# neptune-ai/open-solution-mapping-challenge

Measured on NVIDIA H100. Metric: 300x300 tiles/sec fwd+bwd ResNet101-UNet, higher is better.
Workload: dtype bf16

## Files before the change

### open-solution-mapping-challenge_b200/csrc/conv_gemm.cu

```cuda
#include "host_common.h"
#include "conv_gemm.cuh"
#include "../../include/mcb200.h"
#include <algorithm>
#include <mutex>
#include <stdlib.h>

namespace mcb {

static void pick_tile(int Wv, int Hv, int N, int max_rows, int row_mult, int* pbw, int* pbh, int* pbn) {
  double best = -1.0;
  int bbw = 1, bbh = 1, bbn = 1;
  for (int bw = 1; bw <= std::min(max_rows, std::min(Wv, 256)); ++bw) {
    for (int bh = 1; bw * bh <= max_rows && bh <= std::min(Hv, 256); ++bh) {
      const int bn_max = std::min(256, max_rows / (bw * bh));
      for (int bn = 1; bn <= bn_max; ++bn) {
        if (bn > N && row_mult == 1) break;
        const int rows = bw * bh * bn;
        if (rows % row_mult != 0) continue;
        const long tiles = (long)((Wv + bw - 1) / bw) * ((Hv + bh - 1) / bh) * ((N + bn - 1) / bn);
        const double eff = (double)Wv * Hv * N / ((double)tiles * max_rows);
        const double score = eff + 1e-6 * bw + 1e-9 * bh;
        if (score > best) {
          best = score;
          bbw = bw; bbh = bh; bbn = bn;
        }
      }
    }
  }
  *pbw = bbw; *pbh = bbh; *pbn = bbn;
}

constexpr int kSmemBudget = 227 * 1024;
constexpr int kMaxStagesHalo = 9, kMaxStages = 6;
constexpr int kTwoStagingMinStages = 3;
constexpr int kHaloMinChannels = 128;
constexpr int kBn256MinWaveX10 = 6;
constexpr int kWgradWavesX10 = 10;
constexpr int kWgradMinKb = 6;
constexpr int kWgradKbTarget = 64;
constexpr int kWgradMinWaveX10 = 4;

struct TestHooks { int force_bn, halo, wgrad_splits; };
static TestHooks test_hooks() {
  auto get = [](const char* name, int dflt) {
    const char* v = getenv(name);
    return v ? atoi(v) : dflt;
  };
  return {get("MCB_FORCE_BN", 0), get("MCB_HALO", 2), get("MCB_WGRAD_SPLITS", 0)};
}

template <int BN, int BK, bool B_MN, bool HALO>
static int launch_conv_inst(const ConvGemmParams& p, dim3 grid, size_t smem, cudaStream_t st) {
  static bool attr_set = false;
  if (!attr_set) {
    MCB_CHECK_CUDA(cudaFuncSetAttribute(conv_gemm_kernel<BN, BK, B_MN, HALO>,
                                        cudaFuncAttributeMaxDynamicSharedMemorySize, kSmemBudget));
    attr_set = true;
  }
  conv_gemm_kernel<BN, BK, B_MN, HALO><<<grid, kConvThreads, smem, st>>>(p);
  MCB_LAUNCH_CHECK();
  return MCB_OK;
}

template <int BK, bool B_MN, bool HALO>
static int launch_conv_bn(int BN, const ConvGemmParams& p, dim3 grid, size_t smem, cudaStream_t st) {
  switch (BN) {
    case 256: return launch_conv_inst<256, BK, B_MN, HALO>(p, grid, smem, st);
    case 128: return launch_conv_inst<128, BK, B_MN, HALO>(p, grid, smem, st);
    case 64: return launch_conv_inst<64, BK, B_MN, HALO>(p, grid, smem, st);
    case 32: return launch_conv_inst<32, BK, B_MN, HALO>(p, grid, smem, st);
  }
  return fail(MCB_ERR_UNSUPPORTED, "unsupported BN %d", BN);
}

static int launch_conv(int BN, int BK, bool b_mn, ConvGemmParams& p, int m_tiles, int n_tiles, int phases,
                       cudaStream_t st, bool halo = false) {
  const int a_bytes = halo ? ((kHaloW * kHaloH * BK * 2 + 1023) / 1024) * 1024 : 128 * BK * 2;
  const int b_bytes = BN * BK * 2;
  const int stage = halo ? b_bytes : a_bytes + b_bytes;
  const int out_buf_bytes = 128 * BN * 2;
  const int aux_bytes = p.aux_mode != 0 ? 2 * 128 * (BN >= 64 ? 64 : 32) * 2 : 0;
  const int base = aux_bytes + kStatBytes + 1024  + 1536  + (halo ? 2 * a_bytes : 0);
  const int out_bufs = (kSmemBudget - base - 2 * out_buf_bytes) / stage >= kTwoStagingMinStages ? 2 : 1;
  const int fixed = base + out_bufs * out_buf_bytes;
  const int stages = std::max(2, std::min(halo ? kMaxStagesHalo : kMaxStages, (kSmemBudget - fixed) / stage));
  p.stages = stages;
  p.out_bufs = out_bufs;
  p.m_tiles = m_tiles; p.n_tiles = n_tiles; p.phases = phases;
  const size_t smem = (size_t)stages * stage + fixed;
  const long total = (long)m_tiles * n_tiles * phases;
  dim3 grid((unsigned)std::min<long>(total, num_sms()), 1, 1);
  const int nch = n_tiles * BN;
  const bool red = p.stats != nullptr || p.aux_mode == 2 || (p.aux_mode == 1 && p.bn_dbeta != nullptr);
  p.red_stride = 2 * nch;
  if (red && (long)grid.x * p.red_stride > kConvRedCap)
    return fail(MCB_ERR_UNSUPPORTED, "conv: reduction rows %u x %d exceed the workspace", grid.x, p.red_stride);
  int r;
  if (halo) {
    if (BK == 64) r = b_mn ? launch_conv_bn<64, true, true>(BN, p, grid, smem, st) : launch_conv_bn<64, false, true>(BN, p, grid, smem, st);
    else r = b_mn ? launch_conv_bn<32, true, true>(BN, p, grid, smem, st) : launch_conv_bn<32, false, true>(BN, p, grid, smem, st);
  } else {
    if (BK == 64) r = b_mn ? launch_conv_bn<64, true, false>(BN, p, grid, smem, st) : launch_conv_bn<64, false, false>(BN, p, grid, smem, st);
    else r = b_mn ? launch_conv_bn<32, true, false>(BN, p, grid, smem, st) : launch_conv_bn<32, false, false>(BN, p, grid, smem, st);
  }
  if (r || !red) return r;
  const int rows = (int)grid.x;
  if (p.aux_mode == 0) {
    conv_red_finish_kernel<<<det_finish_grid(2L * nch, rows), kDetFinishThreads, 0, st>>>(
        0L, rows, (long)p.red_stride, 2L * nch, (long)nch, p.stats + p.n_off, (long)p.stats_c);
  } else {
    conv_red_finish_kernel<<<det_finish_grid(nch, rows), kDetFinishThreads, 0, st>>>(
        0L, rows, (long)p.red_stride, (long)nch, (long)nch, p.bn_dbeta + p.n_off, 0L);
    if (p.aux_mode == 2)
      conv_red_finish_kernel<<<det_finish_grid(nch, rows), kDetFinishThreads, 0, st>>>(
          (long)nch, rows, (long)p.red_stride, (long)nch, (long)nch, p.bn_dgamma + p.n_off, 0L);
  }
  MCB_LAUNCH_CHECK();
  return MCB_OK;
}

static bool use_halo(int ksize, int stride, int W, int H, int k_channels) {
  const int mode = test_hooks().halo;
  if (ksize != 3 || stride != 1 || mode == 0) return false;
  if (mode == 2) return k_channels >= kHaloMinChannels && W % 8 == 0 && H % 16 == 0 && W >= 80;
  const double eff = (double)W * H / ((double)((W + 7) / 8) * 8 * ((H + 15) / 16) * 16);
  return eff >= 0.8;
}

static int pick_bn(int n_total, long m_tiles, int phases) {
  int bn = 32;
  for (int cand : {256, 128, 64, 32}) {
    if (n_total % cand == 0) { bn = cand; break; }
  }
  const long sms = num_sms();
  if (bn > 128 && m_tiles * phases * (n_total / bn) * 10 < sms * kBn256MinWaveX10) bn = 128;
  if (bn > 64 && n_total % 64 == 0 && m_tiles * phases * (n_total / bn) < sms / 3) bn = 64;
  const int forced = test_hooks().force_bn;
// ... 340 lines not shown
```

### open-solution-mapping-challenge_b200/csrc/conv_gemm.cuh

```cuda
#pragma once
#include "tc.cuh"
#include "detsum.cuh"

namespace mcb {

constexpr int kMaxTaps = 24;

constexpr long kConvRedCap = 256L * 4096;
constexpr int kWgradRegions = 4;
constexpr long kWgradRegionCap = 4L * 1024 * 1024;
MCB_DET_WORKSPACE(float, g_conv_red, kConvRedCap, conv_red_finish_kernel)
MCB_DET_WORKSPACE(float, g_wgrad_red, kWgradRegions * kWgradRegionCap, wgrad_red_finish_kernel)
constexpr int kGemmThreads = 384;
constexpr int kProducerRegs = 40, kMmaRegs = 232;

struct TapDesc {
  int16_t src;
  int16_t dx, dy;
  int16_t nchunks;
  int32_t wk0;
  int32_t wtap;
};

struct ConvGemmParams {
// ... 32 lines not shown
struct WgradTap {
  int16_t srcA, ax, ay;
  int16_t srcB, bx, by;
  int32_t wtap;
};

struct WgradParams {
  CUtensorMap tmA[4];
  CUtensorMap tmB[4];
  WgradTap taps[16];
  int ntaps;
  int Wv, Hv, Nimg;
  int bw, bh, bn, rows;
  int tiles_x, tiles_y, tiles_total;
  int splits;
  int stages;
  float* dw;
  int cout, cin_total, ci_off;
  int a_cw;
  int a_chunks;
  int cin_src;
  long slice;
  long ws_off;
};

__device__ __forceinline__ uint8_t* align_up_1024(uint8_t* p) {
  const uint32_t a = static_cast<uint32_t>(__cvta_generic_to_shared(p));
  return p + ((1024u - (a & 1023u)) & 1023u);
}


constexpr int kConvThreads = 512;
constexpr int kConvProducerRegs = 24, kConvEpilogueRegs = 120, kConvMmaRegs = 184;

constexpr int kHaloW = 10, kHaloH = 18;

constexpr int kStatBytes = 4 * 8 * 16 * 4;

__device__ __forceinline__ void epi_wg_sync() { asm volatile("bar.sync 1, 128;" ::: "memory"); }

template <int BN, int BK, bool B_MN, bool HALO>
__global__ void __launch_bounds__(kConvThreads, 1) conv_gemm_kernel(const __grid_constant__ ConvGemmParams p) {
  static_assert(BK == 64 || BK == 32, "BK");
  static_assert(BN == 32 || BN == 64 || BN == 128 || BN == 256, "BN");
  constexpr int A_ROW_BYTES = BK * 2;
  constexpr int A_BYTES = HALO ? ((kHaloW * kHaloH * A_ROW_BYTES + 1023) / 1024) * 1024 : 128 * A_ROW_BYTES;
  constexpr int B_BYTES = BN * BK * 2;
  constexpr int STAGE_BYTES = HALO ? B_BYTES : A_BYTES + B_BYTES;
  constexpr int A_RING_BYTES = HALO ? 2 * A_BYTES : 0;
  constexpr uint32_t A_LAYOUT = (BK == 64) ? tc::LAYOUT_SW128 : tc::LAYOUT_SW64;
  constexpr int BMN_CW = (BN >= 64) ? 64 : 32;
  constexpr int BMN_ROW_BYTES = BMN_CW * 2;
  constexpr int BMN_SUB_BYTES = BK * BMN_ROW_BYTES;
  constexpr uint32_t BMN_LAYOUT = (BMN_CW == 64) ? tc::LAYOUT_SW128 : tc::LAYOUT_SW64;
  constexpr int OUT_CW = (BN >= 64) ? 64 : 32;
  constexpr int OUT_ROW_BYTES = OUT_CW * 2;
  constexpr int OUT_CHUNK_BYTES = 128 * OUT_ROW_BYTES;
  constexpr int OUT_CHUNKS = BN / OUT_CW;
  constexpr int OUT_TILE_BYTES = OUT_CHUNKS * OUT_CHUNK_BYTES;
  constexpr int ACC = BN / 2;

  extern __shared__ uint8_t smem_raw[];
  uint8_t* smem = align_up_1024(smem_raw);
  const int stages = p.stages;
  const int out_bufs = p.out_bufs;
  const int aux_mode = p.aux_mode;
  uint8_t* a_ring = smem + (size_t)stages * STAGE_BYTES;
  uint8_t* out_stage = a_ring + A_RING_BYTES;
  uint8_t* aux_stage = out_stage + (size_t)out_bufs * OUT_TILE_BYTES;
  float* stat_scratch = reinterpret_cast<float*>(aux_stage + (aux_mode != 0 ? 2 * OUT_CHUNK_BYTES : 0));
  uint64_t* full_bar = reinterpret_cast<uint64_t*>(reinterpret_cast<uint8_t*>(stat_scratch) + kStatBytes);
  uint64_t* empty_bar = full_bar + stages;
  uint64_t* a_full_bar = empty_bar + stages;
  uint64_t* a_empty_bar = a_full_bar + 2;
  uint64_t* aux_full_bar = a_empty_bar + 2;
  uint64_t* staged_bar = aux_full_bar + 2;
  uint64_t* drained_bar = staged_bar + 2;
  int* row_ok = reinterpret_cast<int*>(drained_bar + 2);

  const int warp = __shfl_sync(0xffffffffu, (int)(threadIdx.x >> 5), 0);
  const int lane = threadIdx.x & 31;
  const int tiles_per_phase = p.m_tiles * p.n_tiles;
  const int total_tiles = tiles_per_phase * p.phases;

  if (warp == 0 && lane == 0) {
    for (int s = 0; s < stages; ++s) {
      tc::mbar_init(&full_bar[s], 1);
      tc::mbar_init(&empty_bar[s], 2);
    }
    tc::mbar_init(&a_full_bar[0], 1);
    tc::mbar_init(&a_full_bar[1], 1);
    tc::mbar_init(&a_empty_bar[0], 2);
    tc::mbar_init(&a_empty_bar[1], 2);
    for (int b = 0; b < 2; ++b) {
      tc::mbar_init(&aux_full_bar[b], 1);
      tc::mbar_init(&staged_bar[b], 8);
      tc::mbar_init(&drained_bar[b], 1);
    }
    tc::fence_barrier_init();
    tc::prefetch_tmap(&p.tmB);
    tc::prefetch_tmap(&p.tmA[0]);
  }
  __syncthreads();

  if (warp < 4) {
    tc::regs_dealloc<kConvProducerRegs>();
    if (warp != 0) return;
    const uint32_t a_bytes = (uint32_t)p.rows * A_ROW_BYTES;
    uint32_t ag = 0;
    int ring_s = 0;
    uint32_t ring_ph = 0;
    for (int t = blockIdx.x; t < total_tiles; t += gridDim.x) {
      const int phase_id = t % p.phases;
      const int mt = (t / p.phases) % p.m_tiles;
      const int nt = t / (p.phases * p.m_tiles);
      const int tx = mt % p.tiles_x, ty = (mt / p.tiles_x) % p.tiles_y, tn = mt / (p.tiles_x * p.tiles_y);
      const int x0 = tx * p.bw, y0 = ty * p.bh, n0 = tn * p.bn;
      const int ncol0 = nt * BN;
      const int tap_begin = p.tap_start[phase_id], tap_end = tap_begin + p.tap_count[phase_id];
      auto load_b = [&](uint8_t* sb, uint64_t* bar, const TapDesc& tap, int ch) {
        if (!B_MN) {
          tc::tma_load_3d(sb, &p.tmB, bar, tap.wk0 + ch * BK, p.n_off + ncol0, tap.wtap);
        } else {
#pragma unroll
          for (int j = 0; j < BN / BMN_CW; ++j)
            tc::tma_load_3d(sb + j * BMN_SUB_BYTES, &p.tmB, bar, p.n_off + ncol0 + j * BMN_CW, tap.wk0 + ch * BK,
                            tap.wtap);
        }
      };
      if (HALO) {
        const int nsrc = (tap_end - tap_begin) / 9;
        for (int sidx = 0; sidx < nsrc; ++sidx) {
          const TapDesc t0 = p.taps[tap_begin + sidx];
          for (int ch = 0; ch < t0.nchunks; ++ch, ++ag) {
            const int as = ag & 1;
            tc::mbar_wait(&a_empty_bar[as], ((ag >> 1) & 1) ^ 1);
            if (tc::elect_one()) {
              tc::mbar_expect_tx(&a_full_bar[as], (uint32_t)(kHaloW * kHaloH * A_ROW_BYTES));
              tc::tma_load_4d(a_ring + (size_t)as * A_BYTES, &p.tmA[t0.src], &a_full_bar[as], ch * BK, x0 - 1, y0 - 1, n0);
// ... 4 lines not shown
              const uint32_t ph = ring_ph;
              if (++ring_s == stages) { ring_s = 0; ring_ph ^= 1; }
              tc::mbar_wait(&empty_bar[s], ph ^ 1);
              uint8_t* sb = smem + (size_t)s * STAGE_BYTES;
              if (tc::elect_one()) {
                tc::mbar_expect_tx(&full_bar[s], B_BYTES);
                load_b(sb, &full_bar[s], tap, ch);
              }
            }
          }
        }
        continue;
      }
      for (int tp = tap_begin; tp < tap_end; ++tp) {
        const TapDesc tap = p.taps[tp];
        const CUtensorMap* mA = &p.tmA[tap.src];
        for (int ch = 0; ch < tap.nchunks; ++ch) {
          const int s = ring_s;
          const uint32_t ph = ring_ph;
          if (++ring_s == stages) { ring_s = 0; ring_ph ^= 1; }
          tc::mbar_wait(&empty_bar[s], ph ^ 1);
          uint8_t* sa = smem + (size_t)s * STAGE_BYTES;
          if (tc::elect_one()) {
            tc::mbar_expect_tx(&full_bar[s], a_bytes + B_BYTES);
            tc::tma_load_4d(sa, mA, &full_bar[s], ch * BK, x0 + tap.dx, y0 + tap.dy, n0);
            load_b(sa + A_BYTES, &full_bar[s], tap, ch);
          }
        }
      }
    }
    return;
  }

  if (warp >= 12) {
    tc::regs_dealloc<kConvEpilogueRegs>();
    const int wtid = threadIdx.x & 127;
    const int ww = wtid >> 5;
    constexpr int CGc = OUT_CW / 8;
    constexpr int RGc = 128 / CGc;
    constexpr int ROWSc = 128 / RGc;
    const bool do_red = (p.stats != nullptr || aux_mode == 2 || (aux_mode == 1 && p.bn_dbeta != nullptr));
    const bool pass2 = do_red || aux_mode != 0;
    float racc1[OUT_CHUNKS], racc2[OUT_CHUNKS];
#pragma unroll
    for (int j = 0; j < OUT_CHUNKS; ++j) racc1[j] = racc2[j] = 0.f;
    int racc_nt = -1;
    uint32_t aux_q = 0;
    auto issue_aux = [&](int t2, int chunk2, int slot) {
      t2 += (chunk2 / OUT_CHUNKS) * (int)gridDim.x;
      chunk2 %= OUT_CHUNKS;
      if (t2 >= total_tiles) return;
      const int ph2 = t2 % p.phases;
      const int mt2 = (t2 / p.phases) % p.m_tiles;
      const int nt2 = t2 / (p.phases * p.m_tiles);
      const int tx2 = mt2 % p.tiles_x, ty2 = (mt2 / p.tiles_x) % p.tiles_y, tn2 = mt2 / (p.tiles_x * p.tiles_y);
      tc::mbar_expect_tx(&aux_full_bar[slot], (uint32_t)p.rows * OUT_ROW_BYTES);
      tc::tma_load_4d(aux_stage + (size_t)slot * OUT_CHUNK_BYTES, &p.tmX[ph2], &aux_full_bar[slot],
                      p.n_off + nt2 * BN + chunk2 * OUT_CW, tx2 * p.bw, ty2 * p.bh, tn2 * p.bn);
    };
    if (aux_mode != 0 && wtid == 0) {
      issue_aux(blockIdx.x, 0, 0);
      issue_aux(blockIdx.x, 1, 1);
    }
    float* red_row = g_conv_red + (size_t)blockIdx.x * p.red_stride;
    const int red_half = p.red_stride >> 1;
    if (do_red)
      for (int i = wtid; i < p.red_stride; i += 128) red_row[i] = 0.f;
    auto flush_reductions = [&]() {
      if (racc_nt >= 0 && wtid < OUT_CW) {
#pragma unroll
        for (int j = 0; j < OUT_CHUNKS; ++j) {
          const int ch = racc_nt * BN + j * OUT_CW + wtid;
          red_row[ch] += racc1[j];
          red_row[red_half + ch] += racc2[j];
          racc1[j] = racc2[j] = 0.f;
        }
      }
    };

    int it = 0;
    for (int t = blockIdx.x; t < total_tiles; t += gridDim.x, ++it) {
      const int phase_id = t % p.phases;
      const int mt = (t / p.phases) % p.m_tiles;
      const int nt = t / (p.phases * p.m_tiles);
      const int tx = mt % p.tiles_x, ty = (mt / p.tiles_x) % p.tiles_y, tn = mt / (p.tiles_x * p.tiles_y);
      const int x0 = tx * p.bw, y0 = ty * p.bh, n0 = tn * p.bn;
      const int ncol0 = nt * BN;
      const bool tile_full = p.rows == 128 && x0 + p.bw <= p.Wv && y0 + p.bh <= p.Hv && n0 + p.bn <= p.Nimg;
      if (do_red && nt != racc_nt) {
        flush_reductions();
        racc_nt = nt;
      }
      if (pass2 && !tile_full) {
        const int wi = wtid % p.bw, hi = (wtid / p.bw) % p.bh, ni = wtid / (p.bw * p.bh);
        row_ok[wtid] = wtid < p.rows && x0 + wi < p.Wv && y0 + hi < p.Hv && n0 + ni < p.Nimg;
      }
      const int b = it % out_bufs;
      tc::mbar_wait(&staged_bar[b], (uint32_t)(it / out_bufs) & 1);
      uint8_t* obuf = out_stage + (size_t)b * OUT_TILE_BYTES;

#pragma unroll 1
      for (int chunk = 0; chunk < OUT_CHUNKS; ++chunk) {
        uint8_t* cbuf = obuf + (size_t)chunk * OUT_CHUNK_BYTES;
        const int aslot = aux_q & 1;
        if (pass2) {
          epi_wg_sync();
          const uint8_t* abuf = aux_stage + (size_t)aslot * OUT_CHUNK_BYTES;
          if (aux_mode != 0) tc::mbar_wait(&aux_full_bar[aslot], (aux_q >> 1) & 1);
          const bool bnred = aux_mode == 2;
          const int cg = wtid % CGc, rg = wtid / CGc;
          const int ch0 = p.n_off + ncol0 + chunk * OUT_CW + cg * 8;
          float s1[8], s2[8], mu[8], is[8], sc[8], sh[8];
#pragma unroll
          for (int j = 0; j < 8; ++j) s1[j] = s2[j] = mu[j] = is[j] = sc[j] = sh[j] = 0.f;
          if (bnred) {
#pragma unroll
            for (int j = 0; j < 8; ++j) {
              mu[j] = __ldg(p.bn_mean + ch0 + j);
              is[j] = __ldg(p.bn_invstd + ch0 + j);
              sc[j] = __ldg(p.bn_gamma + ch0 + j) * is[j];
              sh[j] = __ldg(p.bn_beta + ch0 + j) - mu[j] * sc[j];
            }
          }
          const uint32_t row0_off = (uint32_t)(rg * ROWSc) * OUT_ROW_BYTES;
          const int swz_rg = (OUT_CW == 64) ? 0 : (rg & 1) * 2;
#pragma unroll
          for (int rr = 0; rr < ROWSc; ++rr) {
            if (!tile_full && !row_ok[rg * ROWSc + rr]) continue;
            const int unit = (OUT_CW == 64) ? (cg ^ rr) : (cg ^ (swz_rg + (rr >> 1)));
            const uint32_t off = row0_off + (uint32_t)rr * OUT_ROW_BYTES + (uint32_t)unit * 16;
            const uint4 pk = *reinterpret_cast<const uint4*>(cbuf + off);
            const __nv_bfloat162* h2 = reinterpret_cast<const __nv_bfloat162*>(&pk);
            if (aux_mode == 0) {
#pragma unroll
              for (int j = 0; j < 4; ++j) {
                const float2 xy = __bfloat1622float2(h2[j]);
                s1[2 * j] += xy.x; s2[2 * j] += xy.x * xy.x;
                s1[2 * j + 1] += xy.y; s2[2 * j + 1] += xy.y * xy.y;
              }
            } else if (aux_mode == 1) {
              const uint4 ak = *reinterpret_cast<const uint4*>(abuf + off);
              const uint32_t w[4] = {ak.x, ak.y, ak.z, ak.w};
              uint32_t o[4] = {pk.x, pk.y, pk.z, pk.w};
#pragma unroll
              for (int e = 0; e < 4; ++e) {
                const uint32_t lo = w[e] & 0xFFFFu, hi2 = w[e] >> 16;
                if (!(lo != 0 && lo < 0x8000u)) o[e] &= 0xFFFF0000u;
                if (!(hi2 != 0 && hi2 < 0x8000u)) o[e] &= 0x0000FFFFu;
              }
              *reinterpret_cast<uint4*>(cbuf + off) = make_uint4(o[0], o[1], o[2], o[3]);
              if (do_red) {
#pragma unroll
                for (int e = 0; e < 4; ++e) {
                  s1[2 * e] += __uint_as_float(o[e] << 16);
                  s1[2 * e + 1] += __uint_as_float(o[e] & 0xFFFF0000u);
                }
              }
            } else {
              const uint4 zk = *reinterpret_cast<const uint4*>(abuf + off);
              const __nv_bfloat162* z2 = reinterpret_cast<const __nv_bfloat162*>(&zk);
              uint32_t o[4] = {pk.x, pk.y, pk.z, pk.w};
#pragma unroll
              for (int j = 0; j < 4; ++j) {
                float2 g = __bfloat1622float2(h2[j]);
                const float2 zz = __bfloat1622float2(z2[j]);
                if (!(fmaf(zz.x, sc[2 * j], sh[2 * j]) > 0.f)) { g.x = 0.f; o[j] &= 0xFFFF0000u; }
                if (!(fmaf(zz.y, sc[2 * j + 1], sh[2 * j + 1]) > 0.f)) { g.y = 0.f; o[j] &= 0x0000FFFFu; }
                s1[2 * j] += g.x; s2[2 * j] += g.x * ((zz.x - mu[2 * j]) * is[2 * j]);
                s1[2 * j + 1] += g.y; s2[2 * j + 1] += g.y * ((zz.y - mu[2 * j + 1]) * is[2 * j + 1]);
              }
              *reinterpret_cast<uint4*>(cbuf + off) = make_uint4(o[0], o[1], o[2], o[3]);
            }
          }
          if (aux_mode != 0) tc::fence_proxy_async_smem();
          if (do_red) {
#pragma unroll
            for (int off = CGc; off < 32; off <<= 1) {
#pragma unroll
              for (int j = 0; j < 8; ++j) {
                s1[j] += __shfl_xor_sync(0xffffffffu, s1[j], off);
                s2[j] += __shfl_xor_sync(0xffffffffu, s2[j], off);
              }
            }
            if (lane < CGc) {
              float4* scq = reinterpret_cast<float4*>(stat_scratch + ((size_t)ww * CGc + lane) * 16);
              scq[0] = make_float4(s1[0], s2[0], s1[1], s2[1]);
              scq[1] = make_float4(s1[2], s2[2], s1[3], s2[3]);
              scq[2] = make_float4(s1[4], s2[4], s1[5], s2[5]);
              scq[3] = make_float4(s1[6], s2[6], s1[7], s2[7]);
            }
          }
          epi_wg_sync();
          if (do_red && wtid < OUT_CW) {
            float a1 = 0.f, a2 = 0.f;
#pragma unroll
            for (int w4 = 0; w4 < 4; ++w4) {
              const float2 v2 = *reinterpret_cast<const float2*>(stat_scratch + ((size_t)w4 * CGc + (wtid >> 3)) * 16 + (wtid & 7) * 2);
              a1 += v2.x;
              a2 += v2.y;
            }
#pragma unroll
            for (int j = 0; j < OUT_CHUNKS; ++j)
              if (j == chunk) { racc1[j] += a1; racc2[j] += a2; }
          }
        }

        if (wtid == 0) {
          const CUtensorMap* mD = &p.tmD[phase_id];
          if (p.accumulate) tc::tma_reduce_add_4d(mD, cbuf, p.n_off + ncol0 + chunk * OUT_CW, x0, y0, n0);
          else tc::tma_store_4d(mD, cbuf, p.n_off + ncol0 + chunk * OUT_CW, x0, y0, n0);
          if (aux_mode != 0) issue_aux(t, chunk + 2, aslot);
        }
        ++aux_q;
      }
      if (wtid == 0) {
        tc::tma_store_commit();
        tc::tma_store_wait_read0();
        tc::mbar_arrive(&drained_bar[b]);
      }
    }
    if (do_red) flush_reductions();
    return;
  }

  tc::regs_alloc<kConvMmaRegs>();
  const int wg = (warp >> 2) - 1;
  const int wtid = threadIdx.x & 127;
  const int r_lo = wg * 64 + (wtid >> 5) * 16 + (lane >> 2);

  float acc[ACC];
#pragma unroll
  for (int i = 0; i < ACC; ++i) acc[i] = 0.f;
  uint32_t ag = 0;
  int ring_s = 0;
  uint32_t ring_ph = 0;
  int it = 0;
  for (int t = blockIdx.x; t < total_tiles; t += gridDim.x, ++it) {
    const int phase_id = t % p.phases;
    const int tap_begin = p.tap_start[phase_id], tap_end = tap_begin + p.tap_count[phase_id];
    {
      int prev_s = -1, prev_as = -1;
      auto release_prev = [&]() {
        if (wtid == 0) {
          if (prev_s >= 0) tc::mbar_arrive(&empty_bar[prev_s]);
          if (prev_as >= 0) tc::mbar_arrive(&a_empty_bar[prev_as]);
        }
      };
      auto mma_block = [&](uint64_t da0, uint64_t db0, bool first) {
        tc::wgmma_fence();
#pragma unroll
        for (int k = 0; k < BK / 16; ++k) {
          const uint64_t da = da0 + (uint64_t)((k * 32) >> 4);
          const uint64_t db = B_MN ? db0 + (uint64_t)((k * 16 * BMN_ROW_BYTES) >> 4) : db0 + (uint64_t)((k * 32) >> 4);
          if constexpr (BN == 256) {
            constexpr uint32_t B_HALF = B_MN ? 2 * BMN_SUB_BYTES : 128 * A_ROW_BYTES;
            tc::wgmma_bf16<128, 0, B_MN ? 1 : 0>(*reinterpret_cast<float(*)[64]>(acc), da, db, (!first || k > 0) ? 1u : 0u);
            tc::wgmma_bf16<128, 0, B_MN ? 1 : 0>(*reinterpret_cast<float(*)[64]>(acc + 64), da, db + (B_HALF >> 4),
                                                 (!first || k > 0) ? 1u : 0u);
          } else {
            tc::wgmma_bf16<BN, 0, B_MN ? 1 : 0>(acc, da, db, (!first || k > 0) ? 1u : 0u);
          }
        }
        tc::wgmma_commit();
        tc::wgmma_wait<1>();
        release_prev();
      };
      auto b_desc = [&](uint32_t sb) {
        return B_MN ? tc::make_smem_desc(sb, BMN_SUB_BYTES, 8 * BMN_ROW_BYTES, BMN_LAYOUT)
                    : tc::make_smem_desc(sb, 16, 8 * A_ROW_BYTES, A_LAYOUT);
      };
      if (HALO) {
        const int nsrc = (tap_end - tap_begin) / 9;
        int i = 0;
        for (int sidx = 0; sidx < nsrc; ++sidx) {
          const int nch = p.taps[tap_begin + sidx].nchunks;
          for (int ch = 0; ch < nch; ++ch, ++ag) {
            const int as = ag & 1;
            tc::mbar_wait(&a_full_bar[as], (ag >> 1) & 1);
            const uint32_t a_base = tc::smem_u32(a_ring + (size_t)as * A_BYTES) + (uint32_t)(wg * 8 * kHaloW * A_ROW_BYTES);
            for (int tt = 0; tt < 9; ++tt, ++i) {
              const TapDesc tap = p.taps[tap_begin + tt * nsrc + sidx];
              const int s = ring_s;
              const uint32_t ph = ring_ph;
              if (++ring_s == stages) { ring_s = 0; ring_ph ^= 1; }
              tc::mbar_wait(&full_bar[s], ph);
              const uint32_t sa = a_base + (uint32_t)(((1 + tap.dy) * kHaloW + (1 + tap.dx)) * A_ROW_BYTES);
              mma_block(tc::make_smem_desc(sa, 16, kHaloW * A_ROW_BYTES, A_LAYOUT),
                        b_desc(tc::smem_u32(smem + (size_t)s * STAGE_BYTES)), i == 0);
              prev_s = s;
              prev_as = (tt == 8) ? as : -1;
            }
          }
        }
      } else {
        int num_kb = 0;
        for (int tp = tap_begin; tp < tap_end; ++tp) num_kb += p.taps[tp].nchunks;
        for (int i = 0; i < num_kb; ++i) {
          const int s = ring_s;
          const uint32_t ph = ring_ph;
          if (++ring_s == stages) { ring_s = 0; ring_ph ^= 1; }
          tc::mbar_wait(&full_bar[s], ph);
          const uint32_t sa = tc::smem_u32(smem + (size_t)s * STAGE_BYTES);
          mma_block(tc::make_smem_desc(sa + (uint32_t)(wg * 64 * A_ROW_BYTES), 16, 8 * A_ROW_BYTES, A_LAYOUT),
                    b_desc(sa + A_BYTES), i == 0);
          prev_s = s;
        }
      }
      tc::wgmma_wait<0>();
      tc::fence_acc(acc);
      release_prev();
    }

    const int mt = (t / p.phases) % p.m_tiles;
    const int nt = t / (p.phases * p.m_tiles);
    const int tx = mt % p.tiles_x, ty = (mt / p.tiles_x) % p.tiles_y, tn = mt / (p.tiles_x * p.tiles_y);
    const int x0 = tx * p.bw, y0 = ty * p.bh, n0 = tn * p.bn;
    const int ncol0 = nt * BN;
    const int b = it % out_bufs;
    tc::mbar_wait(&drained_bar[b], ((uint32_t)(it / out_bufs) & 1) ^ 1);
    uint8_t* obuf = out_stage + (size_t)b * OUT_TILE_BYTES;
#pragma unroll
    for (int h = 0; h < 2; ++h) {
      const int row = r_lo + 8 * h;
      const __nv_bfloat16* rrow = nullptr;
      if (p.residual != nullptr) {
        const int wi = row % p.bw, hi = (row / p.bw) % p.bh, ni = row / (p.bw * p.bh);
        const int ox = x0 + wi, oy = y0 + hi, on = n0 + ni;
        if (row < p.rows && ox < p.Wv && oy < p.Hv && on < p.Nimg) {
          const int fy = oy * p.mask_s + (p.mask_s == 2 ? (phase_id >> 1) : 0);
          const int fx = ox * p.mask_s + (p.mask_s == 2 ? (phase_id & 1) : 0);
          rrow = p.residual + (size_t)((on * p.mask_H + fy) * p.mask_W + fx) * p.mask_C + p.n_off + ncol0;
        }
      }
      uint8_t* rowp = obuf + (size_t)row * OUT_ROW_BYTES;
      const int swz = (OUT_CW == 64) ? (row & 7) : ((row >> 1) & 3);
#pragma unroll
      for (int j = 0; j < BN / 8; ++j) {
        const int col = 8 * j + 2 * (lane & 3);
        float v0 = acc[4 * j + 2 * h], v1 = acc[4 * j + 2 * h + 1];
        if (p.scale != nullptr) {
          const float2 sv = __ldg(reinterpret_cast<const float2*>(p.scale + p.n_off + ncol0 + col));
          v0 *= sv.x; v1 *= sv.y;
        }
        if (p.bias != nullptr) {
          const float2 bv = __ldg(reinterpret_cast<const float2*>(p.bias + p.n_off + ncol0 + col));
          v0 += bv.x; v1 += bv.y;
        }
        if (rrow != nullptr) {
          const float2 rv = __bfloat1622float2(*reinterpret_cast<const __nv_bfloat162*>(rrow + col));
          v0 += rv.x; v1 += rv.y;
        }
        if (p.relu) { v0 = fmaxf(v0, 0.f); v1 = fmaxf(v1, 0.f); }
        constexpr int UNITS = OUT_CW / 8;
        const int chunk = j / UNITS, unit = (j % UNITS) ^ swz;
        *reinterpret_cast<uint32_t*>(rowp + (size_t)chunk * OUT_CHUNK_BYTES + unit * 16 + 4 * (lane & 3)) =
            tc::pack_bf16x2(v0, v1);
      }
    }
    tc::fence_proxy_async_smem();
    __syncwarp();
    if (lane == 0) tc::mbar_arrive(&staged_bar[b]);
  }
}

template <int BN>
__global__ void __launch_bounds__(kGemmThreads, 1) wgrad_kernel(const __grid_constant__ WgradParams p) {
  static_assert(BN == 32 || BN == 64 || BN == 128 || BN == 256, "BN");
  constexpr int KROWS = 64;
  constexpr int B_CW = (BN >= 64) ? 64 : 32;
  constexpr int B_ROW_BYTES = B_CW * 2;
  constexpr int B_SUB_BYTES = KROWS * B_ROW_BYTES;
  constexpr int B_SUBS = BN / B_CW;
  constexpr int B_BYTES = B_SUBS * B_SUB_BYTES;
  constexpr uint32_t B_LAYOUT = (B_CW == 64) ? tc::LAYOUT_SW128 : tc::LAYOUT_SW64;
  constexpr int A_SUB_BYTES = KROWS * 128;
  constexpr int A_BYTES = 2 * A_SUB_BYTES;
  constexpr int STAGE_BYTES = A_BYTES + B_BYTES;

  extern __shared__ uint8_t smem_raw[];
  uint8_t* smem = align_up_1024(smem_raw);
  const int stages = p.stages;
  uint64_t* full_bar = reinterpret_cast<uint64_t*>(smem + (size_t)stages * STAGE_BYTES);
  uint64_t* empty_bar = full_bar + stages;

  const int warp = __shfl_sync(0xffffffffu, (int)(threadIdx.x >> 5), 0);
  const int lane = threadIdx.x & 31;
  const int ncol0 = blockIdx.x * BN;
  const int m0 = blockIdx.y * 128;
  const int tap_id = blockIdx.z / p.splits;
  const int split = blockIdx.z % p.splits;
  const WgradTap tap = p.taps[tap_id];
  const int per = (p.tiles_total + p.splits - 1) / p.splits;
  const int kb_begin = split * per;
  const int kb_end = min(p.tiles_total, kb_begin + per);
// ... 107 lines not shown
```

Baseline: 1006.

## Add inline-epilogue conv kernel variant without a dedicated epilogue warpgroup for short CTAs

```diff
diff --git a/open-solution-mapping-challenge_b200/csrc/conv_gemm.cu b/open-solution-mapping-challenge_b200/csrc/conv_gemm.cu
--- a/open-solution-mapping-challenge_b200/csrc/conv_gemm.cu
+++ b/open-solution-mapping-challenge_b200/csrc/conv_gemm.cu
@@ -33,6 +33,7 @@
 constexpr int kSmemBudget = 227 * 1024;
 constexpr int kMaxStagesHalo = 9, kMaxStages = 6;
 constexpr int kTwoStagingMinStages = 3;
+constexpr int kInlineEpilogueMaxTilesPerCta = 4;
 constexpr int kHaloMinChannels = 128;
 constexpr int kBn256MinWaveX10 = 6;
 constexpr int kWgradWavesX10 = 10;
@@ -49,28 +50,39 @@
   return {get("MCB_FORCE_BN", 0), get("MCB_HALO", 2), get("MCB_WGRAD_SPLITS", 0)};
 }
 
-template <int BN, int BK, bool B_MN, bool HALO>
+template <int BN, int BK, bool B_MN, bool HALO, bool EPI_WG>
 static int launch_conv_inst(const ConvGemmParams& p, dim3 grid, size_t smem, cudaStream_t st) {
   static bool attr_set = false;
   if (!attr_set) {
-    MCB_CHECK_CUDA(cudaFuncSetAttribute(conv_gemm_kernel<BN, BK, B_MN, HALO>,
+    MCB_CHECK_CUDA(cudaFuncSetAttribute(conv_gemm_kernel<BN, BK, B_MN, HALO, EPI_WG>,
                                         cudaFuncAttributeMaxDynamicSharedMemorySize, kSmemBudget));
     attr_set = true;
   }
-  conv_gemm_kernel<BN, BK, B_MN, HALO><<<grid, kConvThreads, smem, st>>>(p);
+  conv_gemm_kernel<BN, BK, B_MN, HALO, EPI_WG><<<grid, EPI_WG ? kConvThreads : kGemmThreads, smem, st>>>(p);
   MCB_LAUNCH_CHECK();
   return MCB_OK;
 }
 
-template <int BK, bool B_MN, bool HALO>
+template <int BK, bool B_MN, bool HALO, bool EPI_WG>
 static int launch_conv_bn(int BN, const ConvGemmParams& p, dim3 grid, size_t smem, cudaStream_t st) {
   switch (BN) {
-    case 256: return launch_conv_inst<256, BK, B_MN, HALO>(p, grid, smem, st);
-    case 128: return launch_conv_inst<128, BK, B_MN, HALO>(p, grid, smem, st);
-    case 64: return launch_conv_inst<64, BK, B_MN, HALO>(p, grid, smem, st);
-    case 32: return launch_conv_inst<32, BK, B_MN, HALO>(p, grid, smem, st);
+    case 256: return launch_conv_inst<256, BK, B_MN, HALO, EPI_WG>(p, grid, smem, st);
+    case 128: return launch_conv_inst<128, BK, B_MN, HALO, EPI_WG>(p, grid, smem, st);
+    case 64: return launch_conv_inst<64, BK, B_MN, HALO, EPI_WG>(p, grid, smem, st);
+    case 32: return launch_conv_inst<32, BK, B_MN, HALO, EPI_WG>(p, grid, smem, st);
   }
   return fail(MCB_ERR_UNSUPPORTED, "unsupported BN %d", BN);
+}
+
+template <bool EPI_WG>
+static int launch_conv_layout(int BN, int BK, bool b_mn, bool halo, const ConvGemmParams& p, dim3 grid, size_t smem,
+                              cudaStream_t st) {
+  if (halo) {
+    if (BK == 64) return b_mn ? launch_conv_bn<64, true, true, EPI_WG>(BN, p, grid, smem, st) : launch_conv_bn<64, false, true, EPI_WG>(BN, p, grid, smem, st);
+    return b_mn ? launch_conv_bn<32, true, true, EPI_WG>(BN, p, grid, smem, st) : launch_conv_bn<32, false, true, EPI_WG>(BN, p, grid, smem, st);
+  }
+  if (BK == 64) return b_mn ? launch_conv_bn<64, true, false, EPI_WG>(BN, p, grid, smem, st) : launch_conv_bn<64, false, false, EPI_WG>(BN, p, grid, smem, st);
+  return b_mn ? launch_conv_bn<32, true, false, EPI_WG>(BN, p, grid, smem, st) : launch_conv_bn<32, false, false, EPI_WG>(BN, p, grid, smem, st);
 }
 
 static int launch_conv(int BN, int BK, bool b_mn, ConvGemmParams& p, int m_tiles, int n_tiles, int phases,
@@ -78,31 +90,36 @@
   const int a_bytes = halo ? ((kHaloW * kHaloH * BK * 2 + 1023) / 1024) * 1024 : 128 * BK * 2;
   const int b_bytes = BN * BK * 2;
   const int stage = halo ? b_bytes : a_bytes + b_bytes;
+  const long total = (long)m_tiles * n_tiles * phases;
+  dim3 grid((unsigned)std::min<long>(total, num_sms()), 1, 1);
+  const long per_cta = (total + grid.x - 1) / grid.x;
+  const bool epi_wg = per_cta > kInlineEpilogueMaxTilesPerCta;
   const int out_buf_bytes = 128 * BN * 2;
   const int aux_bytes = p.aux_mode != 0 ? 2 * 128 * (BN >= 64 ? 64 : 32) * 2 : 0;
-  const int base = aux_bytes + kStatBytes + 1024  + 1536  + (halo ? 2 * a_bytes : 0);
-  const int out_bufs = (kSmemBudget - base - 2 * out_buf_bytes) / stage >= kTwoStagingMinStages ? 2 : 1;
-  const int fixed = base + out_bufs * out_buf_bytes;
-  const int stages = std::max(2, std::min(halo ? kMaxStagesHalo : kMaxStages, (kSmemBudget - fixed) / stage));
+  const int base = aux_bytes + (epi_wg ? 1 : 2) * kStatBytes + 1024  + 1536  +
+                   (halo ? 2 * a_bytes : 0);
+  const int max_stages = halo ? kMaxStagesHalo : kMaxStages;
+  int out_bufs, stages;
+  if (epi_wg) {
+    out_bufs = (kSmemBudget - base - 2 * out_buf_bytes) / stage >= kTwoStagingMinStages ? 2 : 1;
+  } else {
+    out_bufs = per_cta == 1 ? 0 : 1;
+  }
+  stages = std::max(2, std::min(max_stages, (kSmemBudget - base - out_bufs * out_buf_bytes) / stage));
+  if (out_bufs == 0 && stages * stage < out_buf_bytes)
+    return fail(MCB_ERR_UNSUPPORTED, "conv: operand ring %d B below the %d B staging buffer", stages * stage,
+                out_buf_bytes);
   p.stages = stages;
   p.out_bufs = out_bufs;
   p.m_tiles = m_tiles; p.n_tiles = n_tiles; p.phases = phases;
-  const size_t smem = (size_t)stages * stage + fixed;
-  const long total = (long)m_tiles * n_tiles * phases;
-  dim3 grid((unsigned)std::min<long>(total, num_sms()), 1, 1);
+  const size_t smem = (size_t)stages * stage + base + out_bufs * out_buf_bytes;
   const int nch = n_tiles * BN;
   const bool red = p.stats != nullptr || p.aux_mode == 2 || (p.aux_mode == 1 && p.bn_dbeta != nullptr);
   p.red_stride = 2 * nch;
   if (red && (long)grid.x * p.red_stride > kConvRedCap)
     return fail(MCB_ERR_UNSUPPORTED, "conv: reduction rows %u x %d exceed the workspace", grid.x, p.red_stride);
-  int r;
-  if (halo) {
-    if (BK == 64) r = b_mn ? launch_conv_bn<64, true, true>(BN, p, grid, smem, st) : launch_conv_bn<64, false, true>(BN, p, grid, smem, st);
-    else r = b_mn ? launch_conv_bn<32, true, true>(BN, p, grid, smem, st) : launch_conv_bn<32, false, true>(BN, p, grid, smem, st);
-  } else {
-    if (BK == 64) r = b_mn ? launch_conv_bn<64, true, false>(BN, p, grid, smem, st) : launch_conv_bn<64, false, false>(BN, p, grid, smem, st);
-    else r = b_mn ? launch_conv_bn<32, true, false>(BN, p, grid, smem, st) : launch_conv_bn<32, false, false>(BN, p, grid, smem, st);
-  }
+  const int r = epi_wg ? launch_conv_layout<true>(BN, BK, b_mn, halo, p, grid, smem, st)
+                       : launch_conv_layout<false>(BN, BK, b_mn, halo, p, grid, smem, st);
   if (r || !red) return r;
   const int rows = (int)grid.x;
   if (p.aux_mode == 0) {
diff --git a/open-solution-mapping-challenge_b200/csrc/conv_gemm.cuh b/open-solution-mapping-challenge_b200/csrc/conv_gemm.cuh
--- a/open-solution-mapping-challenge_b200/csrc/conv_gemm.cuh
+++ b/open-solution-mapping-challenge_b200/csrc/conv_gemm.cuh
@@ -88,15 +88,134 @@
 
 constexpr int kConvThreads = 512;
 constexpr int kConvProducerRegs = 24, kConvEpilogueRegs = 120, kConvMmaRegs = 184;
+constexpr int kConvInlineProducerRegs = 24, kConvInlineMmaRegs = 240;
 
 constexpr int kHaloW = 10, kHaloH = 18;
 
 constexpr int kStatBytes = 4 * 8 * 16 * 4;
 
-__device__ __forceinline__ void epi_wg_sync() { asm volatile("bar.sync 1, 128;" ::: "memory"); }
-
-template <int BN, int BK, bool B_MN, bool HALO>
-__global__ void __launch_bounds__(kConvThreads, 1) conv_gemm_kernel(const __grid_constant__ ConvGemmParams p) {
+constexpr int kEpiBar = 1, kMmaPairBar = 2, kMmaWgBar = 3;
+__device__ __forceinline__ void wg_sync(int bar) { asm volatile("bar.sync %0, 128;" ::"r"(bar) : "memory"); }
+__device__ __forceinline__ void mma_pair_sync() { asm volatile("bar.sync %0, 256;" ::"n"(kMmaPairBar) : "memory"); }
+
+template <int OUT_CW>
+__device__ __forceinline__ void conv_pass2_chunk(const ConvGemmParams& p, bool pass2, bool do_red, int bar, int wtid,
+                                                 uint8_t* cbuf, const uint8_t* abuf, uint64_t* aux_bar, uint32_t aux_par,
+                                                 float* scratch, bool tile_full, const int* row_ok, int phase_id,
+                                                 int chan0, int x0, int y0, int n0, float& a1, float& a2) {
+  constexpr int OUT_ROW_BYTES = OUT_CW * 2;
+  constexpr int CGc = OUT_CW / 8;
+  constexpr int RGc = 128 / CGc;
+  constexpr int ROWSc = 128 / RGc;
+  const int aux_mode = p.aux_mode;
+  const int lane = wtid & 31, ww = wtid >> 5;
+  if (pass2) {
+    wg_sync(bar);
+    if (aux_mode != 0) tc::mbar_wait(aux_bar, aux_par);
+    const bool bnred = aux_mode == 2;
+    const int cg = wtid % CGc, rg = wtid / CGc;
+    const int ch0 = chan0 + cg * 8;
+    float s1[8], s2[8], mu[8], is[8], sc[8], sh[8];
+#pragma unroll
+    for (int j = 0; j < 8; ++j) s1[j] = s2[j] = mu[j] = is[j] = sc[j] = sh[j] = 0.f;
+    if (bnred) {
+#pragma unroll
+      for (int j = 0; j < 8; ++j) {
+        mu[j] = __ldg(p.bn_mean + ch0 + j);
+        is[j] = __ldg(p.bn_invstd + ch0 + j);
+        sc[j] = __ldg(p.bn_gamma + ch0 + j) * is[j];
+        sh[j] = __ldg(p.bn_beta + ch0 + j) - mu[j] * sc[j];
+      }
+    }
+    const uint32_t row0_off = (uint32_t)(rg * ROWSc) * OUT_ROW_BYTES;
+    const int swz_rg = (OUT_CW == 64) ? 0 : (rg & 1) * 2;
+#pragma unroll
+    for (int rr = 0; rr < ROWSc; ++rr) {
+      if (!tile_full && !row_ok[rg * ROWSc + rr]) continue;
+      const int unit = (OUT_CW == 64) ? (cg ^ rr) : (cg ^ (swz_rg + (rr >> 1)));
+      const uint32_t off = row0_off + (uint32_t)rr * OUT_ROW_BYTES + (uint32_t)unit * 16;
+      const uint4 pk = *reinterpret_cast<const uint4*>(cbuf + off);
+      const __nv_bfloat162* h2 = reinterpret_cast<const __nv_bfloat162*>(&pk);
+      if (aux_mode == 0) {
+#pragma unroll
+        for (int j = 0; j < 4; ++j) {
+          const float2 xy = __bfloat1622float2(h2[j]);
+          s1[2 * j] += xy.x; s2[2 * j] += xy.x * xy.x;
+          s1[2 * j + 1] += xy.y; s2[2 * j + 1] += xy.y * xy.y;
+        }
+      } else if (aux_mode == 1) {
+        const uint4 ak = *reinterpret_cast<const uint4*>(abuf + off);
+        const uint32_t w[4] = {ak.x, ak.y, ak.z, ak.w};
+        uint32_t o[4] = {pk.x, pk.y, pk.z, pk.w};
+#pragma unroll
+        for (int e = 0; e < 4; ++e) {
+          const uint32_t lo = w[e] & 0xFFFFu, hi2 = w[e] >> 16;
+          if (!(lo != 0 && lo < 0x8000u)) o[e] &= 0xFFFF0000u;
+          if (!(hi2 != 0 && hi2 < 0x8000u)) o[e] &= 0x0000FFFFu;
+        }
+        *reinterpret_cast<uint4*>(cbuf + off) = make_uint4(o[0], o[1], o[2], o[3]);
+        if (do_red) {
+#pragma unroll
+          for (int e = 0; e < 4; ++e) {
+            s1[2 * e] += __uint_as_float(o[e] << 16);
+            s1[2 * e + 1] += __uint_as_float(o[e] & 0xFFFF0000u);
+          }
+        }
+      } else {
+        const uint4 zk = *reinterpret_cast<const uint4*>(abuf + off);
+        const __nv_bfloat162* z2 = reinterpret_cast<const __nv_bfloat162*>(&zk);
+        uint32_t o[4] = {pk.x, pk.y, pk.z, pk.w};
+#pragma unroll
+        for (int j = 0; j < 4; ++j) {
+          float2 g = __bfloat1622float2(h2[j]);
+          const float2 zz = __bfloat1622float2(z2[j]);
+          if (!(fmaf(zz.x, sc[2 * j], sh[2 * j]) > 0.f)) { g.x = 0.f; o[j] &= 0xFFFF0000u; }
+          if (!(fmaf(zz.y, sc[2 * j + 1], sh[2 * j + 1]) > 0.f)) { g.y = 0.f; o[j] &= 0x0000FFFFu; }
+          s1[2 * j] += g.x; s2[2 * j] += g.x * ((zz.x - mu[2 * j]) * is[2 * j]);
+          s1[2 * j + 1] += g.y; s2[2 * j + 1] += g.y * ((zz.y - mu[2 * j + 1]) * is[2 * j + 1]);
+        }
+        *reinterpret_cast<uint4*>(cbuf + off) = make_uint4(o[0], o[1], o[2], o[3]);
+      }
+    }
+    if (aux_mode != 0) tc::fence_proxy_async_smem();
+    if (do_red) {
+#pragma unroll
+      for (int off = CGc; off < 32; off <<= 1) {
+#pragma unroll
+        for (int j = 0; j < 8; ++j) {
+          s1[j] += __shfl_xor_sync(0xffffffffu, s1[j], off);
+          s2[j] += __shfl_xor_sync(0xffffffffu, s2[j], off);
+        }
+      }
+      if (lane < CGc) {
+        float4* scq = reinterpret_cast<float4*>(scratch + ((size_t)ww * CGc + lane) * 16);
+        scq[0] = make_float4(s1[0], s2[0], s1[1], s2[1]);
+        scq[1] = make_float4(s1[2], s2[2], s1[3], s2[3]);
+        scq[2] = make_float4(s1[4], s2[4], s1[5], s2[5]);
+        scq[3] = make_float4(s1[6], s2[6], s1[7], s2[7]);
+      }
+    }
+    wg_sync(bar);
+    if (do_red && wtid < OUT_CW) {
+      a1 = 0.f; a2 = 0.f;
+#pragma unroll
+      for (int w4 = 0; w4 < 4; ++w4) {
+        const float2 v2 = *reinterpret_cast<const float2*>(scratch + ((size_t)w4 * CGc + (wtid >> 3)) * 16 + (wtid & 7) * 2);
+        a1 += v2.x;
+        a2 += v2.y;
+      }
+    }
+  }
+  if (wtid == 0) {
+    const CUtensorMap* mD = &p.tmD[phase_id];
+    if (p.accumulate) tc::tma_reduce_add_4d(mD, cbuf, chan0, x0, y0, n0);
+    else tc::tma_store_4d(mD, cbuf, chan0, x0, y0, n0);
+  }
+}
+
+template <int BN, int BK, bool B_MN, bool HALO, bool EPI_WG>
+__global__ void __launch_bounds__(EPI_WG ? kConvThreads : kGemmThreads, 1)
+    conv_gemm_kernel(const __grid_constant__ ConvGemmParams p) {
   static_assert(BK == 64 || BK == 32, "BK");
   static_assert(BN == 32 || BN == 64 || BN == 128 || BN == 256, "BN");
   constexpr int A_ROW_BYTES = BK * 2;
@@ -122,10 +241,11 @@
   const int out_bufs = p.out_bufs;
   const int aux_mode = p.aux_mode;
   uint8_t* a_ring = smem + (size_t)stages * STAGE_BYTES;
-  uint8_t* out_stage = a_ring + A_RING_BYTES;
-  uint8_t* aux_stage = out_stage + (size_t)out_bufs * OUT_TILE_BYTES;
+  uint8_t* out_stage = out_bufs == 0 ? smem : a_ring + A_RING_BYTES;
+  uint8_t* aux_stage = a_ring + A_RING_BYTES + (size_t)out_bufs * OUT_TILE_BYTES;
   float* stat_scratch = reinterpret_cast<float*>(aux_stage + (aux_mode != 0 ? 2 * OUT_CHUNK_BYTES : 0));
-  uint64_t* full_bar = reinterpret_cast<uint64_t*>(reinterpret_cast<uint8_t*>(stat_scratch) + kStatBytes);
+  constexpr int STAT_TABLES = EPI_WG ? 1 : 2;
+  uint64_t* full_bar = reinterpret_cast<uint64_t*>(reinterpret_cast<uint8_t*>(stat_scratch) + STAT_TABLES * kStatBytes);
   uint64_t* empty_bar = full_bar + stages;
   uint64_t* a_full_bar = empty_bar + stages;
   uint64_t* a_empty_bar = a_full_bar + 2;
@@ -159,8 +279,21 @@
   }
   __syncthreads();
 
+  auto issue_aux = [&](int t2, int chunk2, int slot) {
+    t2 += (chunk2 / OUT_CHUNKS) * (int)gridDim.x;
+    chunk2 %= OUT_CHUNKS;
+    if (t2 >= total_tiles) return;
+    const int ph2 = t2 % p.phases;
+    const int mt2 = (t2 / p.phases) % p.m_tiles;
+    const int nt2 = t2 / (p.phases * p.m_tiles);
+    const int tx2 = mt2 % p.tiles_x, ty2 = (mt2 / p.tiles_x) % p.tiles_y, tn2 = mt2 / (p.tiles_x * p.tiles_y);
+    tc::mbar_expect_tx(&aux_full_bar[slot], (uint32_t)p.rows * OUT_ROW_BYTES);
+    tc::tma_load_4d(aux_stage + (size_t)slot * OUT_CHUNK_BYTES, &p.tmX[ph2], &aux_full_bar[slot],
+                    p.n_off + nt2 * BN + chunk2 * OUT_CW, tx2 * p.bw, ty2 * p.bh, tn2 * p.bn);
+  };
+
   if (warp < 4) {
-    tc::regs_dealloc<kConvProducerRegs>();
+    tc::regs_dealloc<EPI_WG ? kConvProducerRegs : kConvInlineProducerRegs>();
     if (warp != 0) return;
     const uint32_t a_bytes = (uint32_t)p.rows * A_ROW_BYTES;
     uint32_t ag = 0;
@@ -231,38 +364,23 @@
     return;
   }
 
-  if (warp >= 12) {
+  const bool do_red = (p.stats != nullptr || aux_mode == 2 || (aux_mode == 1 && p.bn_dbeta != nullptr));
+  const bool pass2 = do_red || aux_mode != 0;
+  float* red_row = g_conv_red + (size_t)blockIdx.x * p.red_stride;
+  const int red_half = p.red_stride >> 1;
+
+  if (EPI_WG && warp >= 12) {
     tc::regs_dealloc<kConvEpilogueRegs>();
     const int wtid = threadIdx.x & 127;
-    const int ww = wtid >> 5;
-    constexpr int CGc = OUT_CW / 8;
-    constexpr int RGc = 128 / CGc;
-    constexpr int ROWSc = 128 / RGc;
-    const bool do_red = (p.stats != nullptr || aux_mode == 2 || (aux_mode == 1 && p.bn_dbeta != nullptr));
-    const bool pass2 = do_red || aux_mode != 0;
     float racc1[OUT_CHUNKS], racc2[OUT_CHUNKS];
 #pragma unroll
     for (int j = 0; j < OUT_CHUNKS; ++j) racc1[j] = racc2[j] = 0.f;
     int racc_nt = -1;
     uint32_t aux_q = 0;
-    auto issue_aux = [&](int t2, int chunk2, int slot) {
-      t2 += (chunk2 / OUT_CHUNKS) * (int)gridDim.x;
-      chunk2 %= OUT_CHUNKS;
-      if (t2 >= total_tiles) return;
-      const int ph2 = t2 % p.phases;
-      const int mt2 = (t2 / p.phases) % p.m_tiles;
-      const int nt2 = t2 / (p.phases * p.m_tiles);
-      const int tx2 = mt2 % p.tiles_x, ty2 = (mt2 / p.tiles_x) % p.tiles_y, tn2 = mt2 / (p.tiles_x * p.tiles_y);
-      tc::mbar_expect_tx(&aux_full_bar[slot], (uint32_t)p.rows * OUT_ROW_BYTES);
-      tc::tma_load_4d(aux_stage + (size_t)slot * OUT_CHUNK_BYTES, &p.tmX[ph2], &aux_full_bar[slot],
-                      p.n_off + nt2 * BN + chunk2 * OUT_CW, tx2 * p.bw, ty2 * p.bh, tn2 * p.bn);
-    };
     if (aux_mode != 0 && wtid == 0) {
       issue_aux(blockIdx.x, 0, 0);
       issue_aux(blockIdx.x, 1, 1);
     }
-    float* red_row = g_conv_red + (size_t)blockIdx.x * p.red_stride;
-    const int red_half = p.red_stride >> 1;
     if (do_red)
       for (int i = wtid; i < p.red_stride; i += 128) red_row[i] = 0.f;
     auto flush_reductions = [&]() {
@@ -300,116 +418,18 @@
 
 #pragma unroll 1
       for (int chunk = 0; chunk < OUT_CHUNKS; ++chunk) {
-        uint8_t* cbuf = obuf + (size_t)chunk * OUT_CHUNK_BYTES;
         const int aslot = aux_q & 1;
-        if (pass2) {
-          epi_wg_sync();
-          const uint8_t* abuf = aux_stage + (size_t)aslot * OUT_CHUNK_BYTES;
-          if (aux_mode != 0) tc::mbar_wait(&aux_full_bar[aslot], (aux_q >> 1) & 1);
-          const bool bnred = aux_mode == 2;
-          const int cg = wtid % CGc, rg = wtid / CGc;
-          const int ch0 = p.n_off + ncol0 + chunk * OUT_CW + cg * 8;
-          float s1[8], s2[8], mu[8], is[8], sc[8], sh[8];
-#pragma unroll
-          for (int j = 0; j < 8; ++j) s1[j] = s2[j] = mu[j] = is[j] = sc[j] = sh[j] = 0.f;
-          if (bnred) {
-#pragma unroll
-            for (int j = 0; j < 8; ++j) {
-              mu[j] = __ldg(p.bn_mean + ch0 + j);
-              is[j] = __ldg(p.bn_invstd + ch0 + j);
-              sc[j] = __ldg(p.bn_gamma + ch0 + j) * is[j];
-              sh[j] = __ldg(p.bn_beta + ch0 + j) - mu[j] * sc[j];
-            }
-          }
-          const uint32_t row0_off = (uint32_t)(rg * ROWSc) * OUT_ROW_BYTES;
-          const int swz_rg = (OUT_CW == 64) ? 0 : (rg & 1) * 2;
-#pragma unroll
-          for (int rr = 0; rr < ROWSc; ++rr) {
-            if (!tile_full && !row_ok[rg * ROWSc + rr]) continue;
-            const int unit = (OUT_CW == 64) ? (cg ^ rr) : (cg ^ (swz_rg + (rr >> 1)));
-            const uint32_t off = row0_off + (uint32_t)rr * OUT_ROW_BYTES + (uint32_t)unit * 16;
-            const uint4 pk = *reinterpret_cast<const uint4*>(cbuf + off);
-            const __nv_bfloat162* h2 = reinterpret_cast<const __nv_bfloat162*>(&pk);
-            if (aux_mode == 0) {
-#pragma unroll
-              for (int j = 0; j < 4; ++j) {
-                const float2 xy = __bfloat1622float2(h2[j]);
-                s1[2 * j] += xy.x; s2[2 * j] += xy.x * xy.x;
-                s1[2 * j + 1] += xy.y; s2[2 * j + 1] += xy.y * xy.y;
-              }
-            } else if (aux_mode == 1) {
-              const uint4 ak = *reinterpret_cast<const uint4*>(abuf + off);
-              const uint32_t w[4] = {ak.x, ak.y, ak.z, ak.w};
-              uint32_t o[4] = {pk.x, pk.y, pk.z, pk.w};
-#pragma unroll
-              for (int e = 0; e < 4; ++e) {
-                const uint32_t lo = w[e] & 0xFFFFu, hi2 = w[e] >> 16;
-                if (!(lo != 0 && lo < 0x8000u)) o[e] &= 0xFFFF0000u;
-                if (!(hi2 != 0 && hi2 < 0x8000u)) o[e] &= 0x0000FFFFu;
-              }
-              *reinterpret_cast<uint4*>(cbuf + off) = make_uint4(o[0], o[1], o[2], o[3]);
-              if (do_red) {
-#pragma unroll
-                for (int e = 0; e < 4; ++e) {
-                  s1[2 * e] += __uint_as_float(o[e] << 16);
-                  s1[2 * e + 1] += __uint_as_float(o[e] & 0xFFFF0000u);
-                }
-              }
-            } else {
-              const uint4 zk = *reinterpret_cast<const uint4*>(abuf + off);
-              const __nv_bfloat162* z2 = reinterpret_cast<const __nv_bfloat162*>(&zk);
-              uint32_t o[4] = {pk.x, pk.y, pk.z, pk.w};
-#pragma unroll
-              for (int j = 0; j < 4; ++j) {
-                float2 g = __bfloat1622float2(h2[j]);
-                const float2 zz = __bfloat1622float2(z2[j]);
-                if (!(fmaf(zz.x, sc[2 * j], sh[2 * j]) > 0.f)) { g.x = 0.f; o[j] &= 0xFFFF0000u; }
-                if (!(fmaf(zz.y, sc[2 * j + 1], sh[2 * j + 1]) > 0.f)) { g.y = 0.f; o[j] &= 0x0000FFFFu; }
-                s1[2 * j] += g.x; s2[2 * j] += g.x * ((zz.x - mu[2 * j]) * is[2 * j]);
-                s1[2 * j + 1] += g.y; s2[2 * j + 1] += g.y * ((zz.y - mu[2 * j + 1]) * is[2 * j + 1]);
-              }
-              *reinterpret_cast<uint4*>(cbuf + off) = make_uint4(o[0], o[1], o[2], o[3]);
-            }
-          }
-          if (aux_mode != 0) tc::fence_proxy_async_smem();
-          if (do_red) {
-#pragma unroll
-            for (int off = CGc; off < 32; off <<= 1) {
-#pragma unroll
-              for (int j = 0; j < 8; ++j) {
-                s1[j] += __shfl_xor_sync(0xffffffffu, s1[j], off);
-                s2[j] += __shfl_xor_sync(0xffffffffu, s2[j], off);
-              }
-            }
-            if (lane < CGc) {
-              float4* scq = reinterpret_cast<float4*>(stat_scratch + ((size_t)ww * CGc + lane) * 16);
-              scq[0] = make_float4(s1[0], s2[0], s1[1], s2[1]);
-              scq[1] = make_float4(s1[2], s2[2], s1[3], s2[3]);
-              scq[2] = make_float4(s1[4], s2[4], s1[5], s2[5]);
-              scq[3] = make_float4(s1[6], s2[6], s1[7], s2[7]);
-            }
-          }
-          epi_wg_sync();
-          if (do_red && wtid < OUT_CW) {
-            float a1 = 0.f, a2 = 0.f;
-#pragma unroll
-            for (int w4 = 0; w4 < 4; ++w4) {
-              const float2 v2 = *reinterpret_cast<const float2*>(stat_scratch + ((size_t)w4 * CGc + (wtid >> 3)) * 16 + (wtid & 7) * 2);
-              a1 += v2.x;
-              a2 += v2.y;
-            }
-#pragma unroll
-            for (int j = 0; j < OUT_CHUNKS; ++j)
-              if (j == chunk) { racc1[j] += a1; racc2[j] += a2; }
-          }
-        }
-
-        if (wtid == 0) {
-          const CUtensorMap* mD = &p.tmD[phase_id];
-          if (p.accumulate) tc::tma_reduce_add_4d(mD, cbuf, p.n_off + ncol0 + chunk * OUT_CW, x0, y0, n0);
-          else tc::tma_store_4d(mD, cbuf, p.n_off + ncol0 + chunk * OUT_CW, x0, y0, n0);
-          if (aux_mode != 0) issue_aux(t, chunk + 2, aslot);
-        }
+        float a1, a2;
+        conv_pass2_chunk<OUT_CW>(p, pass2, do_red, kEpiBar, wtid, obuf + (size_t)chunk * OUT_CHUNK_BYTES,
+                                 aux_stage + (size_t)aslot * OUT_CHUNK_BYTES, &aux_full_bar[aslot], (aux_q >> 1) & 1,
+                                 stat_scratch, tile_full, row_ok, phase_id, p.n_off + ncol0 + chunk * OUT_CW, x0, y0,
+                                 n0, a1, a2);
+        if (do_red && wtid < OUT_CW) {
+#pragma unroll
+          for (int j = 0; j < OUT_CHUNKS; ++j)
+            if (j == chunk) { racc1[j] += a1; racc2[j] += a2; }
+        }
+        if (aux_mode != 0 && wtid == 0) issue_aux(t, chunk + 2, aslot);
         ++aux_q;
       }
       if (wtid == 0) {
@@ -422,10 +442,35 @@
     return;
   }
 
-  tc::regs_alloc<kConvMmaRegs>();
+  tc::regs_alloc<EPI_WG ? kConvMmaRegs : kConvInlineMmaRegs>();
   const int wg = (warp >> 2) - 1;
   const int wtid = threadIdx.x & 127;
   const int r_lo = wg * 64 + (wtid >> 5) * 16 + (lane >> 2);
+  constexpr int CH = (OUT_CHUNKS + 1) / 2;
+  const int my_chunks = (OUT_CHUNKS - wg + 1) / 2;
+  float racc1[CH], racc2[CH];
+#pragma unroll
+  for (int j = 0; j < CH; ++j) racc1[j] = racc2[j] = 0.f;
+  int racc_nt = -1;
+  uint32_t aux_n = 0;
+  auto flush_reductions = [&]() {
+    if (racc_nt >= 0 && wtid < OUT_CW) {
+#pragma unroll
+      for (int j = 0; j < CH; ++j) {
+        if (j < my_chunks) {
+          const int ch = racc_nt * BN + (wg + 2 * j) * OUT_CW + wtid;
+          red_row[ch] += racc1[j];
+          red_row[red_half + ch] += racc2[j];
+          racc1[j] = racc2[j] = 0.f;
+        }
+      }
+    }
+  };
+  if constexpr (!EPI_WG) {
+    if (aux_mode != 0 && wtid == 0 && my_chunks > 0) issue_aux(blockIdx.x, wg, wg);
+    if (do_red)
+      for (int i = threadIdx.x - 128; i < p.red_stride; i += 256) red_row[i] = 0.f;
+  }
 
   float acc[ACC];
 #pragma unroll
@@ -451,7 +496,7 @@
         for (int k = 0; k < BK / 16; ++k) {
           const uint64_t da = da0 + (uint64_t)((k * 32) >> 4);
           const uint64_t db = B_MN ? db0 + (uint64_t)((k * 16 * BMN_ROW_BYTES) >> 4) : db0 + (uint64_t)((k * 32) >> 4);
-          if constexpr (BN == 256) {
+          if constexpr (BN == 256 && EPI_WG) {
             constexpr uint32_t B_HALF = B_MN ? 2 * BMN_SUB_BYTES : 128 * A_ROW_BYTES;
             tc::wgmma_bf16<128, 0, B_MN ? 1 : 0>(*reinterpret_cast<float(*)[64]>(acc), da, db, (!first || k > 0) ? 1u : 0u);
             tc::wgmma_bf16<128, 0, B_MN ? 1 : 0>(*reinterpret_cast<float(*)[64]>(acc + 64), da, db + (B_HALF >> 4),
@@ -515,8 +560,14 @@
     const int tx = mt % p.tiles_x, ty = (mt / p.tiles_x) % p.tiles_y, tn = mt / (p.tiles_x * p.tiles_y);
     const int x0 = tx * p.bw, y0 = ty * p.bh, n0 = tn * p.bn;
     const int ncol0 = nt * BN;
-    const int b = it % out_bufs;
-    tc::mbar_wait(&drained_bar[b], ((uint32_t)(it / out_bufs) & 1) ^ 1);
+    int b = 0;
+    if constexpr (EPI_WG) {
+      b = it % out_bufs;
+      tc::mbar_wait(&drained_bar[b], ((uint32_t)(it / out_bufs) & 1) ^ 1);
+    } else {
+      if (wtid == 0) tc::tma_store_wait_read0();
+      mma_pair_sync();
+    }
     uint8_t* obuf = out_stage + (size_t)b * OUT_TILE_BYTES;
 #pragma unroll
     for (int h = 0; h < 2; ++h) {
@@ -557,8 +608,46 @@
       }
     }
     tc::fence_proxy_async_smem();
-    __syncwarp();
-    if (lane == 0) tc::mbar_arrive(&staged_bar[b]);
+    if constexpr (EPI_WG) {
+      __syncwarp();
+      if (lane == 0) tc::mbar_arrive(&staged_bar[b]);
+    } else {
+      const bool tile_full = p.rows == 128 && x0 + p.bw <= p.Wv && y0 + p.bh <= p.Hv && n0 + p.bn <= p.Nimg;
+      if (pass2 && !tile_full && wg == 0) {
+        const int wi = wtid % p.bw, hi = (wtid / p.bw) % p.bh, ni = wtid / (p.bw * p.bh);
+        row_ok[wtid] = wtid < p.rows && x0 + wi < p.Wv && y0 + hi < p.Hv && n0 + ni < p.Nimg;
+      }
+      mma_pair_sync();
+      if (do_red && nt != racc_nt) {
+        flush_reductions();
+        racc_nt = nt;
+      }
+      for (int cj = 0; cj < my_chunks; ++cj) {
+        const int chunk = wg + 2 * cj;
+        float a1, a2;
+        conv_pass2_chunk<OUT_CW>(p, pass2, do_red, kMmaWgBar + wg, wtid, obuf + (size_t)chunk * OUT_CHUNK_BYTES,
+                                 aux_stage + (size_t)wg * OUT_CHUNK_BYTES, &aux_full_bar[wg], aux_n & 1,
+                                 stat_scratch + wg * (kStatBytes / 4), tile_full, row_ok, phase_id,
+                                 p.n_off + ncol0 + chunk * OUT_CW, x0, y0, n0, a1, a2);
+        if (do_red && wtid < OUT_CW) {
+#pragma unroll
+          for (int j = 0; j < CH; ++j)
+            if (j == cj) { racc1[j] += a1; racc2[j] += a2; }
+        }
+        if (aux_mode != 0) {
+          ++aux_n;
+          if (wtid == 0) {
+            if (chunk + 2 < OUT_CHUNKS) issue_aux(t, chunk + 2, wg);
+            else issue_aux(t + (int)gridDim.x, wg, wg);
+          }
+        }
+      }
+      if (wtid == 0) tc::tma_store_commit();
+    }
+  }
+  if constexpr (!EPI_WG) {
+    if (do_red) flush_reductions();
+    if (wtid == 0) tc::tma_store_wait_read0();
   }
 }
 
```

Measured after the change: 1032 (median of 6 runs). +2.5%, better.
